# ZhendongWang6/Uformer

Hardware: AMD Instinct MI355X
Metric: restored images/sec (256x256, Uformer-B) (higher is better)
Workload: dtype bf16

## Files before the change

### include/uformer_hip.h

```cpp
#ifndef UFORMER_HIP_H
#define UFORMER_HIP_H

#include <stddef.h>
#include <stdint.h>

#ifdef __cplusplus
extern "C" {
#endif

#define UF_ABI_VERSION 1

typedef enum { UF_F32 = 0, UF_BF16 = 1, UF_F16 = 2 } uf_dtype;

#define UF_OK 0
#define UF_ERR_SHAPE (-1)
#define UF_ERR_UNSUPPORTED (-2)
#define UF_ERR_ALIGN (-3)
#define UF_ERR_LAUNCH (-4)
#define UF_ERR_WORKSPACE (-5)
#define UF_ERR_NULL (-6)

int uf_version(void);
int uf_last_error(char* buf, size_t n);

// ... 41 lines not shown
int uf_dwconv3x3_gelu_fwd(const void* x, const float* w9, const float* bias, void* out, int B,
                          int H, int W, int C, uf_dtype dtype, void* stream);
int uf_dwconv3x3_fwd(const void* x, const float* w9, const float* bias, void* out, int B, int H,
                     int W, int C, int gelu, uf_dtype dtype, void* stream);

int uf_dwconv3x3_pre_gelu_fwd(const void* x, const float* w9, const float* bias, void* pre_out, void* act_out, int B, int H,
                              int W, int C, uf_dtype dtype, void* stream);
int uf_dwconv3x3_gelu_in_pre_gelu_fwd(const void* pre_in, const float* w9, const float* bias, void* pre_out, void* act_out, int B, int H,
                                      int W, int C, uf_dtype dtype, void* stream);
int uf_dwconv3x3_mul_dgelu(const void* dy, const float* w9_flipped, const void* pre, void* out, int B, int H, int W, int C,
                           uf_dtype dtype, void* stream);

int uf_dwconv_linear2_fwd(const void* h1, const float* w9, const float* bdw, const void* W2_fm,
                          const float* b2, float* x, int ld, int B, int H, int W, int C,
                          uf_dtype dtype, void* stream);

typedef struct uf_block_params {
    const float* norm1_w;
    const float* norm1_b;
    const float* modulator;
    const float* rpb_dense;
    const float* rpb_fm;
    const float* rpb_tab;
    const void* wqkv_fm;
    const float* bqkv;
    const void* wproj;
    const void* wproj_fm;
    const float* bproj;
    const float* norm2_w;
    const float* norm2_b;
// ... 183 lines not shown
int uf_mixup(const float* x, float* out, const float* lam, const int* perm, int B, long long per_sample, void* stream);

typedef struct uf_model_desc {
    int32_t embed_dim, dd_in, in_chans;
    int32_t depths[9];
    const uf_block_params* blocks;
    const float* in_w27;
    const float* in_b;
    const float* out_w;
    const float* out_b;
    const void* down_w[4];
    const float* down_b[4];
    const void* up_w[4];
    const float* up_b[4];
    const void* down_w_fm[4];
} uf_model_desc;

size_t uf_uformer_workspace_bytes(const uf_model_desc* d, int B, int H, int W, uf_dtype dtype);
int uf_uformer_fwd(const uf_model_desc* d, const float* img, float* out, int B, int H, int W,
                   uf_dtype dtype, void* ws, size_t ws_bytes, void* stream);

typedef struct uf_block4_params {
    const float* norm1_w;  const float* norm1_b;  const float* norm2_w;  const float* norm2_b;
    const float* rpb4;
    const void* wqkv;
    const float* bqkv;
    const void* wproj;  const float* bproj;
    const void* w1;     const float* b1;
    const float* wdw9;  const float* bdw;
    const void* w2;     const float* b2;
// ... 46 lines not shown
```

### uformer_amd/_lib.py

```python
from __future__ import annotations

import ctypes as C
import os
import threading

_HERE = os.path.dirname(os.path.abspath(__file__))
LIB_PATH = os.path.join(_HERE, "lib", "libuformer_hip.so")
LIB_PATH = os.environ.get("UFORMER_HIP_LIB", LIB_PATH)

UF_F32, UF_BF16, UF_F16 = 0, 1, 2

c_int, c_void_p, c_size_t, c_float_p = C.c_int, C.c_void_p, C.c_size_t, C.c_void_p


class BlockParams(C.Structure):
    _fields_ = [(n, C.c_void_p) for n in (
        "norm1_w", "norm1_b", "modulator", "rpb_dense", "rpb_fm", "rpb_tab", "wqkv_fm", "bqkv", "wproj", "wproj_fm", "bproj",
        "norm2_w", "norm2_b", "w1_fm", "b1", "wdw9", "bdw", "w2_fm", "b2")] + [
        ("shift", C.c_int32), ("heads", C.c_int32), ("qkv_dw9", C.c_void_p), ("qkv_bdw", C.c_void_p)]


class BlockTrainParams(C.Structure):
    _fields_ = [(n, C.c_void_p) for n in (
        "norm1_w", "norm1_b", "norm2_w", "norm2_b", "modulator", "rpb_dense", "wqkv", "wqkv_t", "bqkv", "wproj", "wproj_t", "bproj",
# ... 14 lines not shown
class Block4Params(C.Structure):
    _fields_ = [(n, C.c_void_p) for n in (
        "norm1_w", "norm1_b", "norm2_w", "norm2_b", "rpb4", "wqkv", "bqkv", "wproj", "bproj", "w1", "b1", "wdw9", "bdw", "w2", "b2")] + [
        ("heads", C.c_int32)]


class ModelDesc(C.Structure):
    _fields_ = [
        ("embed_dim", C.c_int32), ("dd_in", C.c_int32), ("in_chans", C.c_int32),
        ("depths", C.c_int32 * 9),
        ("blocks", C.POINTER(BlockParams)),
        ("in_w27", C.c_void_p), ("in_b", C.c_void_p), ("out_w", C.c_void_p), ("out_b", C.c_void_p),
        ("down_w", C.c_void_p * 4), ("down_b", C.c_void_p * 4),
        ("up_w", C.c_void_p * 4), ("up_b", C.c_void_p * 4),
        ("down_w_fm", C.c_void_p * 4),
    ]


class UnetDesc(C.Structure):
    _fields_ = [
        ("dim", C.c_int32),
        ("in_w27", C.c_void_p), ("in_b", C.c_void_p), ("c11_w1", C.c_void_p), ("c11_b1", C.c_void_p),
        ("w0", C.c_void_p * 9), ("b0", C.c_void_p * 9), ("w2", C.c_void_p * 9), ("b2", C.c_void_p * 9),
        ("w11", C.c_void_p * 9), ("b11", C.c_void_p * 9),
        ("pool_w", C.c_void_p * 4), ("pool_b", C.c_void_p * 4), ("up_w", C.c_void_p * 4), ("up_b", C.c_void_p * 4),
        ("out_w", C.c_void_p), ("out_b", C.c_void_p),
    ]


P = c_void_p
# ... 28 lines not shown
    "uf_linear_residual_fwd": (I, [P, P, P, P, P, P, I, I, I, I, I, I, I, I, P]),
    "uf_layernorm_bwd_workspace_bytes": (c_size_t, [I, I]),
    "uf_layernorm_bwd": (I, [P, I, P, P, I, P, I, P, P, I, I, P, c_size_t, P]),
    "uf_layernorm_bwd_fused": (I, [P, I, P, P, I, I, P, P, I, P, P, I, I, I, I, I, I, I, P, c_size_t, P]),
    "uf_layernorm_bwd_cast": (I, [P, I, P, P, I, I, P, P, I, P, P, I, I, I, I, I, I, I, P, P, I, I, P, c_size_t, P]),
    "uf_linear_wgrad_workspace_bytes": (c_size_t, [I, I, I]),
    "uf_linear_wgrad": (I, [P, I, P, I, P, P, I, I, I, I, P, c_size_t, P]),
    "uf_window_attention_bwd_workspace_bytes": (c_size_t, [I, I]),
    "uf_window_attention_bwd": (I, [P, P, P, P, P, I, P, I, P, P, P, P, I, I, I, I, I, I, I, P, c_size_t, P]),
    "uf_window_attention_bwd_qkv": (I, [P, P, P, P, P, I, P, I, P, P, I, I, I, I, I, I, I, P, c_size_t, P]),
    "uf_dwconv3x3_wgrad_workspace_bytes": (c_size_t, [I, I]),
    "uf_dwconv3x3_wgrad": (I, [P, P, P, P, I, I, I, I, I, P, c_size_t, P]),
    "uf_dwconv3x3_bwd_workspace_bytes": (c_size_t, [I, I]),
    "uf_dwconv3x3_bwd": (I, [P, P, P, P, P, P, I, I, I, I, I, P, c_size_t, P]),
    "uf_dwconv_linear2_fwd": (I, [P, P, P, P, P, P, I, I, I, I, I, I, P]),
    "uf_block_workspace_bytes": (c_size_t, [I, I, I]),
    "uf_lewin_attn_fwd": (I, [C.POINTER(BlockParams), P, I, I, I, I, I, P, I, I, P, c_size_t, P]),
    "uf_leff_fwd": (I, [C.POINTER(BlockParams), P, I, I, I, I, I, I, P, c_size_t, P]),
    "uf_ffn_fwd": (I, [P, I, P, P, P, P, P, P, P, I, I, I, I, P]),
    "uf_mlp_fwd": (I, [C.POINTER(BlockParams), P, I, I, I, I, I, I, P, c_size_t, P]),
    "uf_lewin_attn_train_fwd": (I, [C.POINTER(BlockParams), P, I, P, I, I, I, I, I, P, I, P, P, P, P, P, P, P, P]),
    "uf_lewin_block_fwd": (I, [C.POINTER(BlockParams), P, I, I, I, I, I, P, I, I, P, c_size_t, P]),
    "uf_lewin_block_train_fwd": (I, [C.POINTER(BlockParams), P, I, I, I, I, I, P, P, I, P, c_size_t, P]),
    "uf_downsample_fwd": (I, [P, I, P, P, P, I, I, I, I, I, I, P]),
    "uf_downsample_fm_fwd": (I, [P, I, P, P, P, P, I, I, I, I, I, I, P]),
    "uf_upsample_fwd": (I, [P, I, P, P, P, I, I, I, I, I, I, I, P]),
    "uf_input_proj_fwd": (I, [P, P, P, P, I, I, I, I, I, I, P]),
    "uf_output_proj_fwd": (I, [P, I, P, P, P, P, I, I, I, I, I, P]),
    "uf_rows_sum_workspace_bytes": (c_size_t, [I, I]),
    "uf_rows_sum": (I, [P, I, P, I, I, I, P, c_size_t, P]),
# ... 95 lines not shown
```

### uformer_amd/csrc/uf_attnblk.hip

```cpp
#include <stdlib.h>

#include <atomic>
#include <type_traits>

#include "uf_internal.h"

namespace uf {
namespace {

struct AttnBlkParams {
    float* x; int ld;
    float* xo; int ldo;
    const float* gamma; const float* beta; const float* modulator;
    const void* Wqkv; const float* bqkv;
    const float* rpb_tab;
    const void* Wp; const float* bp;
    const float* gamma2; const float* beta2;
    const void* W1; const float* b1;
    void* h1;
    const float* drop;
    void* s_xn; void* s_q; void* s_k; void* s_vt; void* s_o; void* s_z;
    int n_windows, H, W, shift;
    float qscale;
    float qscale_plain;
// ... 2 lines not shown

constexpr float LOG2E = 1.4426950408889634f;

#ifndef UF_P1_OFFSET
#define UF_P1_OFFSET 0
#endif
#ifndef UF_FC1_OFFSET
#define UF_FC1_OFFSET 0
#endif
#ifndef UF_STAGGER
#define UF_STAGGER 0
#endif
#ifndef UF_SETPRIO
#define UF_SETPRIO 0
#endif
#define UF_PRIO_UP() do { if (UF_SETPRIO) __builtin_amdgcn_s_setprio(1); } while (0)
#define UF_PRIO_DN() do { if (UF_SETPRIO) __builtin_amdgcn_s_setprio(0); } while (0)
#ifndef UF_ABL
#define UF_ABL 0
#endif
#ifndef UF_NT
#define UF_NT 0
#endif
#ifndef UF_LN_ROTATE
#define UF_LN_ROTATE 0
#endif
#ifndef UF_LN_WIDE
#define UF_LN_WIDE 1
#endif
#ifndef UF_QKV_RING
// ... 796 lines not shown
    AttnBlkParams p{};
    p.drop = drop;
    p.x = x; p.ld = ld;
    p.xo = xo ? xo : x; p.ldo = xo ? ldo : ld; p.gamma = bp->norm1_w; p.beta = bp->norm1_b; p.modulator = bp->modulator;
    p.Wqkv = bp->wqkv_fm; p.bqkv = bp->bqkv; p.rpb_tab = bp->rpb_tab;
    p.Wp = bp->wproj_fm; p.bp = bp->bproj;
    p.gamma2 = bp->norm2_w; p.beta2 = bp->norm2_b; p.W1 = bp->w1_fm; p.b1 = bp->b1;
    p.h1 = dtype_half(dtype) ? h1_out : nullptr;
    p.n_windows = B * (H / 8) * (W / 8); p.H = H; p.W = W; p.shift = bp->shift;
    p.qscale = (float)(1.0 / sqrt(32.0)) * LOG2E;
    p.tbuf = debug_get_tbuf();

    const int forced = variant("attn", -1);
    const int lr = (forced >= 0 && forced <= 2) ? forced : (forced == 3 ? 0 : (C == 32 ? 2 : ((C == 128 && p.n_windows >= 4096) ? 1 : 0)));
    const bool st256 = forced == 3;
    const int nt_small = forced == 4 ? 64 : (forced == 5 ? 128 : ((forced < 0 && C == 32 && p.n_windows >= 8192) ? 64 : 0));
#define UF_AB(TT, CV, NTV) return launch_one<TT, CV, NTV>(p, st)
#define UF_AB_HALF(TT)                                                                                                              \
        switch (C) {                                                                                                                    \
            case 32:                                                                                                                    \
                if (nt_small == 64) return launch_one<TT, 32, 64, 0, 0, 4>(p, st);          \
                if (nt_small == 128) return launch_one<TT, 32, 128, 0, 0, 2>(p, st);                     \
                if (lr == 1) return launch_one<TT, 32, 256, 1>(p, st); if (lr == 2) return launch_one<TT, 32, 256, 2>(p, st); UF_AB(TT, 32, 256);      \
            case 64:                                                                                                                    \
                if (nt_small == 64) return launch_one<TT, 64, 64, 0, 0, 4>(p, st);             \
                if (nt_small == 128) return launch_one<TT, 64, 128, 0, 0, 4>(p, st);                            \
                if (lr == 1) return launch_one<TT, 64, 256, 1>(p, st); if (lr == 2) return launch_one<TT, 64, 256, 2>(p, st); UF_AB(TT, 64, 256);      \
            case 128: if (lr == 1) return launch_one<TT, 128, 256, 1>(p, st); if (lr == 2) return launch_one<TT, 128, 256, 2>(p, st); UF_AB(TT, 128, 256);                                                                                              \
            case 256:                                                                                                                   \
                if (p.n_windows <= 256) UF_AB(TT, 256, 512);    \
                if (st256) return launch_one<TT, 256, 256, 3>(p, st);          \
// ... 59 lines not shown
```

### uformer_amd/csrc/uf_internal.h

```cpp
#pragma once
#include "uf_common.h"

namespace uf {

enum ALoad { A_PLAIN = 0, A_FROM_R = 1, A_CONV_DOWN = 2 };
enum Epi {
    E_STORE_T = 0,
    E_STORE_T_GELU = 1,
    E_QKV = 2,
    E_RES_WINREV = 3,
    E_RES = 4,
    E_STORE_R = 5,
    E_UPSAMPLE = 6,
    E_STORE_T_PRE_GELU = 7,
    E_STORE_T_MUL_DGELU = 8
};

struct GemmParams {
    const void* A; int lda;
    const void* W;
    const void* W_fm = nullptr;
    const float* bias;
    int M, N, K;
    int H, W_, C;
// ... 10 lines not shown
int launch_down_dx(const void* dyT, int ld_dy, const void* w_pk_t, void* wc, float* dx, int ld_dx, int B, int H, int W, int Cin, int Cout, int accumulate, uf_dtype dtype,
                   hipStream_t st, bool* done);

constexpr int MAX_SIDE = 7, MAX_LANE_EVENTS = 8;
struct Lane { hipStream_t s[MAX_SIDE] = {}; hipEvent_t fork = nullptr, join[MAX_SIDE] = {}; int n = 0; hipEvent_t ev[MAX_LANE_EVENTS] = {}; int n_ev = 0; };
Lane* acquire_lane(int want, int* dev_out);
void release_lane(Lane* ln, int dev);
bool lane_events(Lane* ln, int want);

void debug_set_tbuf(void* p);
bool attn_block_supported(const uf_block_params* bp, const float* user_mask, uf_dtype dtype, int C, int heads);
int launch_attn_block(const uf_block_params* bp, float* x, int ld, int B, int H, int W, int C, uf_dtype dtype, void* h1_out, hipStream_t st,
                      const float* drop = nullptr, float* xo = nullptr, int ldo = 0);
int launch_leff2(const void* h1, const float* w9, const float* bdw, const void* W2, const float* b2, float* x, int ld, int B, int H, int W, int C,
                 uf_dtype dtype, const float* drop, hipStream_t st);

int launch_attn_block_train(const uf_block_params* bp, const float* x, int ld, float* x1, int ld1, int B, int H, int W, int C, uf_dtype dtype, const float* drop,
                            void* xn, void* q, void* k, void* vt, void* o, void* z, void* a1, hipStream_t st);

}
```

### uformer_amd/csrc/uf_leff2.hip

```cpp
#include <stdlib.h>

#include "uf_internal.h"
#include "uf_mconv.h"

namespace uf {
namespace {

struct Leff2Params {
    const void* h1;
    const float* w9; const float* bdw;
    const void* W2; const float* b2;
    float* x; int ld;
    const float* drop;
    int B, H, W;
    int n_tiles;
    unsigned long long* tbuf;
};

constexpr int KCW = 64;

#ifndef UF_MCONV
#define UF_MCONV 1
#endif
#ifndef UF_LEFF2_CP_DEFAULT
#define UF_LEFF2_CP_DEFAULT false
#endif
template <typename T> __device__ __forceinline__ void cvt8(const char* p, float* f);
template <> __device__ __forceinline__ void cvt8<bf16>(const char* p, float* f) { unpack8<bf16>(*reinterpret_cast<const u32x4*>(p), f); }
template <> __device__ __forceinline__ void cvt8<f16>(const char* p, float* f) { unpack8<f16>(*reinterpret_cast<const u32x4*>(p), f); }
template <> __device__ __forceinline__ void cvt8<float>(const char* p, float* f) {
    const f32x4 a = *reinterpret_cast<const f32x4*>(p), b = *reinterpret_cast<const f32x4*>(p + 16);
    f[0] = a[0]; f[1] = a[1]; f[2] = a[2]; f[3] = a[3]; f[4] = b[0]; f[5] = b[1]; f[6] = b[2]; f[7] = b[3];
}
__device__ __forceinline__ void put8(bf16* p, const float* f) { *reinterpret_cast<u32x4*>(p) = pack8<bf16>(f); }
__device__ __forceinline__ void put8(f16* p, const float* f) { *reinterpret_cast<u32x4*>(p) = pack8<f16>(f); }
__device__ __forceinline__ void put8(float* p, const float* f) {
    *reinterpret_cast<f32x4*>(p) = f32x4{f[0], f[1], f[2], f[3]};
    *reinterpret_cast<f32x4*>(p + 4) = f32x4{f[4], f[5], f[6], f[7]};
}

template <typename T, int C, int NPG, int NC, int NBUF, int WPS, int PW = 4, int CP = 0>
__global__ __launch_bounds__((PW * NPG + NC) * 64, WPS) void leff2_kernel(const Leff2Params p) {
    constexpr int NP = PW * NPG;
    constexpr int MC = sizeof(T) == 2 ? UF_MCONV : 0;
    static_assert(PW == 4 || (PW == 8 && MC != 0), "8 producer waves per group: MFMA stencil only (two pixel tiles per wave)");
    static_assert(CP == 0 || (MC != 0 && PW == 4 && NPG == 1 && NC == 4 * CP), "consumer stencil jobs: MFMA stencil, 4 producers, one job per consumer wave");
    constexpr int PTW = 16 / PW - CP;
    constexpr int SR = 2;
    constexpr int SZ = sizeof(T);
    constexpr int TH = 8, TW = 8, BM = 64;
    constexpr int HID = 4 * C;
    constexpr int KC = KCW * NPG;
    constexpr int NIT = HID / KC;
    static_assert(HID % KC == 0, "interval width");
    constexpr int HW_ = TW + 2, HT = (TH + 2) * HW_;
    constexpr int PS = KCW * SZ;
    constexpr int CPP = PS / 16;
    constexpr int HGB = (HT * PS + 1023) / 1024 * 1024;
    constexpr int NHG = HGB / 1024;
    constexpr int TRB = KC * 4;
    constexpr int TGB = (10 * TRB + 1023) / 1024 * 1024;
    constexpr int NTI = TGB / 1024;
    constexpr int NHI = NPG * NHG;
    constexpr int NI = NHI + NTI;
    constexpr int NS = (NI + NP - 1) / NP;
    constexpr int BUFB = NPG * HGB + TGB;
    constexpr int SAT = KC * SZ + 16;
    constexpr int AT_BYTES = BM * SAT;
    constexpr int WN = (C / 16) < NC ? (C / 16) : NC, WM = NC / WN;
    static_assert(WM <= 4, "consumer grid");
    constexpr int TMW = 4 / WM, TNW = (C / 16) / WN;
    extern __shared__ __attribute__((aligned(16))) char smem[];
    char* Ring = smem;
    char* At0 = smem + NBUF * BUFB;

    const int tid = threadIdx.x, lane = tid & 63;
    const int wave = __builtin_amdgcn_readfirstlane(tid >> 6);
    const bool producer = wave < NP;
    const int fr = lane & 15, fg = lane >> 4;
    const int tiles_x = p.W / TW, tiles_y = p.H / TH;
    const int G = (int)gridDim.x;
    const int nk = (p.n_tiles - (int)blockIdx.x + G - 1) / G;
    const int NTOT = nk * NIT;
    const int bt = xcd_tile(blockIdx.x, p.n_tiles);
    auto tile_coords = [&](int k, int& b, int& y0, int& x0) {
        const int t = xcd_tile((int)blockIdx.x + k * G, p.n_tiles);
// ... 134 lines not shown
    const int wlane = lane * 8 * SZ;
    auto w2_load = [&](int sub, int ks, int slot) {
#pragma unroll
        for (int i = 0; i < TNW; ++i) {
            const int soff = (((wn * TNW + i) * (HID / 32) + sub * 2 + ks) * 64) * 8 * SZ;
            if constexpr (SZ == 2) {
                wf[slot][i].v = __builtin_bit_cast(u32x4, __builtin_amdgcn_raw_buffer_load_b128(wrs, wlane, soff, 0));
            } else {
                wf[slot][i].lo = __builtin_bit_cast(f32x4, __builtin_amdgcn_raw_buffer_load_b128(wrs, wlane, soff, 0));
                wf[slot][i].hi = __builtin_bit_cast(f32x4, __builtin_amdgcn_raw_buffer_load_b128(wrs, wlane + 16, soff, 0));
            }
        }
    };
    auto w2_issue = [&](int sub) {
        if constexpr (WKS == 2) { w2_load(sub, 0, 0); w2_load(sub, 1, 1); }
    };

    f32x4 acc[TNW][TMW];
#pragma unroll
    for (int i = 0; i < TNW; ++i)
#pragma unroll
        for (int j = 0; j < TMW; ++j) acc[i][j] = f32x4{0.f, 0.f, 0.f, 0.f};

    constexpr bool XPRE = SZ == 2 && TNW * TMW <= 4 && CP == 0;
    f32x4 xres[XPRE ? TNW : 1][XPRE ? TMW : 1];
    auto x_ptr = [&](int b, int y0, int x0, int i, int j) -> float* {
        const int n = (wn * TNW + i) * 16 + fg * 4;
        const int pm = (wm * TMW + j) * 16 + fr;
        return p.x + ((size_t)(b * p.H + y0 + (pm >> 3)) * p.W + x0 + (pm & 7)) * p.ld + n;
    };
// ... 22 lines not shown
                for (int ks = 0; ks < 2; ++ks) {
                    if constexpr (WKS == 1) w2_load(sub, ks, 0);
                    Frag<T> af[TMW];
#pragma unroll
                    for (int jj = 0; jj < TMW; ++jj)
                        load_frag(af[jj], reinterpret_cast<const T*>(At + ((wm * TMW + jj) * 16 + fr) * SAT + (g * KCW + ks * 32 + fg * 8) * SZ));
                    __builtin_amdgcn_sched_barrier(0);
#pragma unroll
                    for (int ii = 0; ii < TNW; ++ii)
#pragma unroll
                        for (int jj = 0; jj < TMW; ++jj) mma16(acc[ii][jj], wf[WKS == 2 ? ks : 0][ii], af[jj]);
                    __builtin_amdgcn_sched_barrier(0);
                }
                if (sub + 1 < NIT * NPG) w2_issue(sub + 1);
                else if (j < NTOT) w2_issue(0);
                __builtin_amdgcn_sched_barrier(0);
            }
            if (it == NIT - 1) {
                const float dscale = p.drop ? p.drop[tb] : 1.0f;
#pragma unroll
                for (int i = 0; i < TNW; ++i) {
                    const f32x4 b2 = *reinterpret_cast<const f32x4*>(p.b2 + (wn * TNW + i) * 16 + fg * 4);
#pragma unroll
                    for (int jj = 0; jj < TMW; ++jj) {
                        float* xp = x_ptr(tb, ty0, tx0, i, jj);
                        f32x4 r;
                        if constexpr (XPRE) r = xres[i][jj]; else r = *reinterpret_cast<const f32x4*>(xp);
                        *reinterpret_cast<f32x4*>(xp) = r + (acc[i][jj] + b2) * dscale;
                        acc[i][jj] = f32x4{0.f, 0.f, 0.f, 0.f};
                    }
                }
            }
        }
        if constexpr (CP > 0) {
            if (j < NTOT) {
                const char* Hs = Ring + (j % NBUF) * BUFB;
                const float* Wl = reinterpret_cast<const float*>(Ring + (j % NBUF) * BUFB + NPG * HGB);
                mconv_job<T, MC, 1, KC, SAT, 2 * HW_ * PS>(Hs, Wl, At0 + (j & 1) * AT_BYTES, gq, 4 - CP + (cw >> 2), boff, msk, hshift, fr, fg);
            }
        }
        ct1 = __builtin_readcyclecounter(); ctw += ct1 - ct0; ct0 = ct1;
        lds_barrier();
        ct1 = __builtin_readcyclecounter(); ctbar += ct1 - ct0; ct0 = ct1;
    }
    if (p.tbuf && lane == 0 && (bt & 63) == 0) { p.tbuf[((bt >> 6) * 16 + wave) * 4] = ctw; p.tbuf[((bt >> 6) * 16 + wave) * 4 + 1] = ctbar; p.tbuf[((bt >> 6) * 16 + wave) * 4 + 2] = 0; }
    if (cw == 0 && lane == 0) {
        Census c2 = census;
        if (p.tbuf) { unsigned long long* o = p.tbuf + 65536 + (size_t)bt * 8; o[0] = c2.t0; o[1] = __builtin_readcyclecounter(); o[2] = c2.r0; o[3] = wall_clock64();
            o[4] = (unsigned long long)__builtin_amdgcn_s_getreg((31 << 11) | 4) | ((unsigned long long)__builtin_amdgcn_s_getreg((31 << 11) | 20) << 32); }
    }
}

template <typename T, int C, int NPG, int NC, int NBUF, int WPS, int PW = 4, int CP = 0>
int launch_v(const Leff2Params& p, hipStream_t st) {
    constexpr int SZ = sizeof(T), KC = KCW * NPG;
    constexpr int HGB = (100 * KCW * SZ + 1023) / 1024 * 1024, TGB = (10 * KC * 4 + 1023) / 1024 * 1024;
    constexpr int smem = NBUF * (NPG * HGB + TGB) + 2 * 64 * (KC * SZ + 16) + 1024;
    static_assert(smem <= 160 * 1024, "LDS budget");
    auto kern = leff2_kernel<T, C, NPG, NC, NBUF, WPS, PW, CP>;
    static bool lds_done[64] = {};
    if (int rc = ensure_dynamic_lds(reinterpret_cast<const void*>(kern), smem, lds_done, "leff2")) return rc;
    const long long M = (long long)p.B * p.H * p.W;
    char name[96] = "";
    if (timing_enabled()) snprintf(name, sizeof(name), "leff2_%s_c%d_np%d_nc%d %lldx%dx%d", TypeName<T>::s, C, PW * NPG, NC, M, C, 4 * C);
    {
        ScopedTimer tm(name, 2.0 * M * C * 4 * C + 18.0 * M * 4 * C, (double)M * 4 * C * SZ + (double)M * C * 8, st);
        const int pe = variant("persist", -1);
        const bool pays = C <= 32 || C >= 256 || (C == 128 && p.n_tiles <= 1024);
        const bool persist = pe >= 0 ? pe != 0 : pays;
        constexpr int waves = PW * NPG + NC;
        constexpr int by_lds = (160 * 1024) / smem, by_waves = 32 / waves, by_regs = (WPS * 4) / waves > 0 ? (WPS * 4) / waves : 1;
        constexpr int per_cu = by_lds < by_waves ? (by_lds < by_regs ? by_lds : by_regs) : (by_waves < by_regs ? by_waves : by_regs);
        const int resident = 256 * (per_cu < 1 ? 1 : per_cu);
        int grid = p.n_tiles;
        if (persist && p.n_tiles > resident) {
            const int rounds = (p.n_tiles + resident - 1) / resident;
            grid = ((p.n_tiles + rounds - 1) / rounds + 7) / 8 * 8;
        }
        hipLaunchKernelGGL(kern, dim3((unsigned)grid), dim3(waves * 64), smem, st, p);
    }
    return check_launch("leff2");
}

#ifndef UF_NB512
// ... 33 lines not shown
template <typename T>
int launch_t(const Leff2Params& p, int C, hipStream_t st) {
    switch (C) {
        case 16: return launch_c<T, 16>(p, st);
        case 32: return launch_c<T, 32>(p, st);
        case 64: return launch_c<T, 64>(p, st);
        case 128: return launch_c<T, 128>(p, st);
        case 256: return launch_c<T, 256>(p, st);
        case 512: return launch_c<T, 512>(p, st);
        default:
            set_error("leff2: C=%d unsupported (16,32,64,128,256,512)", C);
            return UF_ERR_UNSUPPORTED;
    }
}

}
unsigned long long* debug_get_tbuf();
}

using namespace uf;

namespace uf {
int launch_leff2(const void* h1, const float* w9, const float* bdw, const void* W2, const float* b2, float* x, int ld, int B, int H, int W, int C,
                 uf_dtype dtype, const float* drop, hipStream_t st) {
    UF_REQUIRE(h1 && w9 && bdw && W2 && b2 && x, UF_ERR_NULL, "uf_dwconv_linear2_fwd: null pointer");
    UF_REQUIRE(B > 0 && H >= 8 && W >= 8 && H % 8 == 0 && W % 8 == 0, UF_ERR_SHAPE, "uf_dwconv_linear2_fwd: B=%d H=%d W=%d (multiples of 8)", B, H, W);
    UF_REQUIRE(ld >= C && ld % 4 == 0, UF_ERR_ALIGN, "uf_dwconv_linear2_fwd: ld=%d", ld);
    UF_REQUIRE(((uintptr_t)h1 % 16) == 0 && ((uintptr_t)W2 % 16) == 0 && ((uintptr_t)x % 16) == 0 && ((uintptr_t)w9 % 16) == 0 &&
                   ((uintptr_t)bdw % 16) == 0 && ((uintptr_t)b2 % 16) == 0,
               UF_ERR_ALIGN, "uf_dwconv_linear2_fwd: operands must be 16-byte aligned");
    UF_REQUIRE((long long)H * W * 4LL * C * (long long)dtype_size(dtype) < 0xffffff00LL, UF_ERR_SHAPE,
               "uf_dwconv_linear2_fwd: one image of the hidden tensor must stay under 4 GiB (32-bit buffer offsets)");
    UF_REQUIRE((long long)B * H * W < 0x7fffffffLL / 4, UF_ERR_SHAPE, "uf_dwconv_linear2_fwd: too many tokens");
    Leff2Params p{};
    p.tbuf = debug_get_tbuf();
    p.h1 = h1; p.w9 = w9; p.bdw = bdw; p.W2 = W2; p.b2 = b2; p.x = x; p.ld = ld; p.B = B; p.H = H; p.W = W; p.drop = drop;
    p.n_tiles = B * (H / 8) * (W / 8);
    if (dtype == UF_BF16) return launch_t<bf16>(p, C, st);
    if (dtype == UF_F16) return launch_t<f16>(p, C, st);
    if (dtype == UF_F32) return launch_t<float>(p, C, st);
    set_error("uf_dwconv_linear2_fwd: dtype %d", (int)dtype);
    return UF_ERR_UNSUPPORTED;
}
}

extern "C" int uf_dwconv_linear2_fwd(const void* h1, const float* w9, const float* bdw, const void* W2, const float* b2,
                                     float* x, int ld, int B, int H, int W, int C, uf_dtype dtype, void* stream) {
    return uf::launch_leff2(h1, w9, bdw, W2, b2, x, ld, B, H, W, C, dtype, nullptr, (hipStream_t)stream);
}
```

### uformer_amd/csrc/uf_model.hip

```cpp
#include <stdlib.h>

#include <mutex>
#include <vector>

#include "uf_internal.h"

namespace uf {

int launch_layernorm(const float* x, int ld_x, const float* gamma, const float* beta, const float* modulator, void* out,
                     int rows, int H, int W, int C, int windowed, int shift, uf_dtype dtype, hipStream_t st);

int launch_unpack_weight_fm(const void* fm, void* w, int N, int K, uf_dtype dtype, hipStream_t st);

namespace {

struct BlockWs {
    char* a;
    char* h1;
    char* h2;
    char* wr;
};

bool wide_block(size_t C) { return C > 512; }

// ... 111 lines not shown
        rc = uf_dwconv3x3_gelu_fwd(w.h1, p->wdw9, p->bdw, w.h2, B, H, W, 4 * C, dtype, st);
        if (rc) return rc;
        rc = launch_unpack_weight_fm(p->w2_fm, w.wr, C, 4 * C, dtype, st);
        if (rc) return rc;
        GemmParams g{};
        g.A = w.h2; g.lda = 4 * C; g.W = w.wr; g.bias = p->b2; g.M = M; g.N = C; g.K = 4 * C;
        g.H = H; g.W_ = W; g.hw = H * W;
        g.out = x; g.ldo = ld; g.resid = x; g.ldr = ld;
        return launch_gemm(g, A_PLAIN, E_RES, dtype, st);
    }
    if (!fc1_done) {
        int rc = uf_ln_linear_gelu_fwd(x, ld, p->norm2_w, p->norm2_b, p->w1_fm, p->b1, w.h1, M, 4 * C, C, dtype, st);
        if (rc) return rc;
    }
    return launch_leff2(w.h1, p->wdw9, p->bdw, p->w2_fm, p->b2, x, ld, B, H, W, C, dtype, drop, st);
}

int block_fwd(const uf_block_params* p, float* x, int ld, int B, int H, int W, int C, const float* user_mask, int n_mask, uf_dtype dtype,
              const BlockWs& w, hipStream_t st, const float* drop_attn, const float* drop_leff) {
    bool fc1_done = false;
    int rc = attn_half(p, x, ld, B, H, W, C, user_mask, n_mask, dtype, w, st, &fc1_done, drop_attn);
    if (rc) return rc;
    return leff_half(p, x, ld, B, H, W, C, dtype, w, st, fc1_done, drop_leff);
}

}
}

using namespace uf;

// ... 172 lines not shown
    UF_REQUIRE(((uintptr_t)ws % 256) == 0, UF_ERR_ALIGN, "uf_uformer_fwd: workspace must be 256-byte aligned");
    UF_REQUIRE(ws_bytes >= pl.total, UF_ERR_WORKSPACE, "uf_uformer_fwd: workspace too small: %zu < %zu", ws_bytes, pl.total);
    UF_REQUIRE(d->in_chans == 3, UF_ERR_UNSUPPORTED, "uf_uformer_fwd: in_chans=%d (3 supported)", d->in_chans);
    hipStream_t st = (hipStream_t)stream;
    char* base = (char*)ws;
    float* D[4];
    for (int k = 0; k < 4; ++k) D[k] = (float*)(base + pl.off_D[k]);
    float* P = (float*)(base + pl.off_P);
    void* bws = base + pl.off_blk;

    auto enc_view = [&](int s, float*& ptr, int& ld) {
        ptr = D[3 - s] + pl.C[s];
        ld = 2 * pl.C[s];
    };
    const uf_block_params* blk = d->blocks;
    auto run_stage = [&](int s, float* x, int ld) -> int {
        for (int i = 0; i < d->depths[s]; ++i, ++blk) {
            int r = (s == 4 && bneck) ? uf_lewin_block4_fwd(bneck + i, x, ld, B, pl.res_h[s], pl.res_w[s], pl.C[s], nullptr, nullptr, dtype, bws, pl.blk_bytes, st)
                                      : uf_lewin_block_fwd(blk, x, ld, B, pl.res_h[s], pl.res_w[s], pl.C[s], nullptr, 0, dtype, bws, pl.blk_bytes, st);
            if (r) return r;
        }
        return UF_OK;
    };

    float* x; int ld;
    enc_view(0, x, ld);
    rc = uf_input_proj_fwd(img, d->in_w27, d->in_b, x, ld, B, d->dd_in, H, W, d->embed_dim, st);
    if (rc) return rc;
    for (int s = 0; s < 4; ++s) {
        rc = run_stage(s, x, ld);
        if (rc) return rc;
        float* nx; int nld;
        if (s < 3) enc_view(s + 1, nx, nld); else { nx = P; nld = pl.C[4]; }
        rc = uf_downsample_fm_fwd(x, ld, d->down_w[s], d->down_w_fm[s], d->down_b[s], nx, nld, B, pl.res_h[s], pl.res_w[s], pl.C[s], dtype, st);
        if (rc) return rc;
        x = nx; ld = nld;
    }
    rc = run_stage(4, x, ld);
    if (rc) return rc;
    for (int k = 0; k < 4; ++k) {
        const int s = 5 + k;
        const int cin = pl.C[s - 1], cout = pl.C[s] / 2;
        rc = uf_upsample_fwd(x, ld, d->up_w[k], d->up_b[k], D[k], pl.C[s], B, pl.res_h[s - 1], pl.res_w[s - 1], cin, cout, dtype, st);
        if (rc) return rc;
        x = D[k]; ld = pl.C[s];
        rc = run_stage(s, x, ld);
        if (rc) return rc;
    }
    return uf_output_proj_fwd(x, ld, d->out_w, d->out_b, img, out, B, H, W, pl.C[8], d->dd_in == 3 ? 1 : 0, st);
}

}

namespace {
int forward_split(const uf_model_desc* d, const uf_block4_params* bneck, const float* img, float* out, int B, int H, int W, uf_dtype dtype,
                  void* ws, size_t ws_bytes, void* stream) {
    static const int env_streams = getenv("UF_STREAMS") ? atoi(getenv("UF_STREAMS")) : 0;
    int n = env_streams > 0 ? (env_streams > MAX_SIDE + 1 ? MAX_SIDE + 1 : env_streams) : (B >= 8 ? 2 : 1);
    if (n > B) n = B;
    if (n < 2 || timing_enabled()) return forward_one_stream(d, bneck, img, out, B, H, W, dtype, ws, ws_bytes, stream);
    UF_REQUIRE(d && img && out && ws, UF_ERR_NULL, "uf_uformer_fwd: null pointer");
// ... 47 lines not shown
```

### uformer_amd/packing.py

```python
from __future__ import annotations

import ctypes as C
from typing import Dict, List

import torch

from . import _lib

Tensor = torch.Tensor


def rpb_dense(table: Tensor, index: Tensor) -> Tensor:
    n = index.shape[0]
    return table.detach()[index.reshape(-1)].reshape(n, n, -1).permute(2, 0, 1).contiguous().float()


def pack_frag(w: Tensor, dtype: torch.dtype) -> Tensor:
    N, K = w.shape
    KP = (K + 31) // 32 * 32
    w = w.detach().to(dtype)
    if KP != K:
        w = torch.nn.functional.pad(w, (0, KP - K))
    return w.reshape(N // 16, 16, KP // 32, 4, 8).permute(0, 2, 3, 1, 4).contiguous()

# ... 167 lines not shown
        }
        for name, tns in g.items():
            setattr(d, name, tns.data_ptr())
        self.keep.append(g)
        for k in range(4):
            dw = pack_downsample(sd[f"dowsample_{k}.conv.0.weight"], dtype)
            db = sd[f"dowsample_{k}.conv.0.bias"].detach().float().clone().contiguous()
            uw = pack_upsample(sd[f"upsample_{k}.deconv.0.weight"], dtype)
            ub = sd[f"upsample_{k}.deconv.0.bias"].detach().float().clone().contiguous()
            d.down_w[k], d.down_b[k], d.up_w[k], d.up_b[k] = dw.data_ptr(), db.data_ptr(), uw.data_ptr(), ub.data_ptr()
            dwf = None
            if dtype in (torch.bfloat16, torch.float16) and dw.is_cuda and dw.shape[0] % 16 == 0 and dw.shape[1] % 32 == 0:
                from . import ops
                dwf = ops.pack_weight_fm(dw)
            d.down_w_fm[k] = dwf.data_ptr() if dwf is not None else None
            self.keep.append((dw, db, uw, ub, dwf))
        self.desc = d


def pack_conv(w: Tensor, dtype: torch.dtype) -> Tensor:
    cout, cin, k, _ = w.shape
    cp, np_ = (cin + 31) // 32 * 32, (cout + 63) // 64 * 64
    t = torch.zeros(np_, k, k, cp, dtype=dtype, device=w.device)
    t[:cout, :, :, :cin] = w.detach().permute(0, 2, 3, 1).to(dtype)
    return t.reshape(np_, -1).contiguous()


def pack_conv_dgrad(w: Tensor, dtype: torch.dtype) -> Tensor:
    return pack_conv(w.detach().transpose(0, 1).flip(2, 3), dtype)


# ... 31 lines not shown
```

Before: 2539.

## Fuse decoder upsample into last block's dwconv+linear2 kernel

Adds a leff2 kernel variant that computes the block's output residual into LDS and then runs the 2x2 transposed-conv upsample GEMM in the same kernel, writing the upsampled tensor directly. This removes the round trip of the stage output through global memory and a separate upsample launch. By default it is enabled only for the C=512, Cout=128 case. It also adds an optional wave-64 attention tile choice for C=64, which is off by default. The fused path skips the write of the block output to x and disables persistent scheduling for this kernel.

```diff
diff --git a/include/uformer_hip.h b/include/uformer_hip.h
--- a/include/uformer_hip.h
+++ b/include/uformer_hip.h
@@ -79,6 +79,9 @@
 int uf_dwconv_linear2_fwd(const void* h1, const float* w9, const float* bdw, const void* W2_fm,
                           const float* b2, float* x, int ld, int B, int H, int W, int C,
                           uf_dtype dtype, void* stream);
+int uf_dwconv_linear2_upsample_fwd(const void* h1, const float* w9, const float* bdw, const void* W2_fm, const float* b2, const float* x, int ld,
+                                   const void* up_w_fm, const float* up_b, float* out, int ld_o, int B, int H, int W, int C, int Cout,
+                                   uf_dtype dtype, void* stream);
 
 typedef struct uf_block_params {
     const float* norm1_w;
@@ -292,6 +295,7 @@
     const void* up_w[4];
     const float* up_b[4];
     const void* down_w_fm[4];
+    const void* up_w_fm[4];
 } uf_model_desc;
 
 size_t uf_uformer_workspace_bytes(const uf_model_desc* d, int B, int H, int W, uf_dtype dtype);
diff --git a/uformer_amd/_lib.py b/uformer_amd/_lib.py
--- a/uformer_amd/_lib.py
+++ b/uformer_amd/_lib.py
@@ -52,6 +52,7 @@
         ("down_w", C.c_void_p * 4), ("down_b", C.c_void_p * 4),
         ("up_w", C.c_void_p * 4), ("up_b", C.c_void_p * 4),
         ("down_w_fm", C.c_void_p * 4),
+        ("up_w_fm", C.c_void_p * 4),
     ]
 
 
@@ -110,6 +111,7 @@
     "uf_dwconv3x3_bwd_workspace_bytes": (c_size_t, [I, I]),
     "uf_dwconv3x3_bwd": (I, [P, P, P, P, P, P, I, I, I, I, I, P, c_size_t, P]),
     "uf_dwconv_linear2_fwd": (I, [P, P, P, P, P, P, I, I, I, I, I, I, P]),
+    "uf_dwconv_linear2_upsample_fwd": (I, [P, P, P, P, P, P, I, P, P, P, I, I, I, I, I, I, I, P]),
     "uf_block_workspace_bytes": (c_size_t, [I, I, I]),
     "uf_lewin_attn_fwd": (I, [C.POINTER(BlockParams), P, I, I, I, I, I, P, I, I, P, c_size_t, P]),
     "uf_leff_fwd": (I, [C.POINTER(BlockParams), P, I, I, I, I, I, I, P, c_size_t, P]),
diff --git a/uformer_amd/csrc/uf_attnblk.hip b/uformer_amd/csrc/uf_attnblk.hip
--- a/uformer_amd/csrc/uf_attnblk.hip
+++ b/uformer_amd/csrc/uf_attnblk.hip
@@ -40,6 +40,9 @@
 #ifndef UF_SETPRIO
 #define UF_SETPRIO 0
 #endif
+#ifndef UF_ATTN_WAVE64
+#define UF_ATTN_WAVE64 0
+#endif
 #define UF_PRIO_UP() do { if (UF_SETPRIO) __builtin_amdgcn_s_setprio(1); } while (0)
 #define UF_PRIO_DN() do { if (UF_SETPRIO) __builtin_amdgcn_s_setprio(0); } while (0)
 #ifndef UF_ABL
@@ -866,7 +869,8 @@
     const int forced = variant("attn", -1);
     const int lr = (forced >= 0 && forced <= 2) ? forced : (forced == 3 ? 0 : (C == 32 ? 2 : ((C == 128 && p.n_windows >= 4096) ? 1 : 0)));
     const bool st256 = forced == 3;
-    const int nt_small = forced == 4 ? 64 : (forced == 5 ? 128 : ((forced < 0 && C == 32 && p.n_windows >= 8192) ? 64 : 0));
+    const bool wave_shape = (C == 32 || (UF_ATTN_WAVE64 && C == 64)) && p.n_windows >= 8192;
+    const int nt_small = forced == 4 ? 64 : (forced == 5 ? 128 : ((forced < 0 && wave_shape) ? 64 : 0));
 #define UF_AB(TT, CV, NTV) return launch_one<TT, CV, NTV>(p, st)
 #define UF_AB_HALF(TT)                                                                                                              \
         switch (C) {                                                                                                                    \
diff --git a/uformer_amd/csrc/uf_internal.h b/uformer_amd/csrc/uf_internal.h
--- a/uformer_amd/csrc/uf_internal.h
+++ b/uformer_amd/csrc/uf_internal.h
@@ -48,6 +48,7 @@
                       const float* drop = nullptr, float* xo = nullptr, int ldo = 0);
 int launch_leff2(const void* h1, const float* w9, const float* bdw, const void* W2, const float* b2, float* x, int ld, int B, int H, int W, int C,
                  uf_dtype dtype, const float* drop, hipStream_t st);
+bool leff2_upsample_supported(int C, int Cout, uf_dtype dtype);
 
 int launch_attn_block_train(const uf_block_params* bp, const float* x, int ld, float* x1, int ld1, int B, int H, int W, int C, uf_dtype dtype, const float* drop,
                             void* xn, void* q, void* k, void* vt, void* o, void* z, void* a1, hipStream_t st);
diff --git a/uformer_amd/csrc/uf_leff2.hip b/uformer_amd/csrc/uf_leff2.hip
--- a/uformer_amd/csrc/uf_leff2.hip
+++ b/uformer_amd/csrc/uf_leff2.hip
@@ -16,6 +16,12 @@
     int n_tiles;
     unsigned long long* tbuf;
 };
+struct Leff2UpParams : Leff2Params {
+    const void* up_w; const float* up_b;
+    float* out; int ld_o;
+};
+template <int UP> struct ParamsOf { typedef Leff2UpParams type; };
+template <> struct ParamsOf<0> { typedef Leff2Params type; };
 
 constexpr int KCW = 64;
 
@@ -39,8 +45,8 @@
     *reinterpret_cast<f32x4*>(p + 4) = f32x4{f[4], f[5], f[6], f[7]};
 }
 
-template <typename T, int C, int NPG, int NC, int NBUF, int WPS, int PW = 4, int CP = 0>
-__global__ __launch_bounds__((PW * NPG + NC) * 64, WPS) void leff2_kernel(const Leff2Params p) {
+template <typename T, int C, int NPG, int NC, int NBUF, int WPS, int PW = 4, int CP = 0, int UP = 0>
+__global__ __launch_bounds__((PW * NPG + NC) * 64, WPS) void leff2_kernel(const typename ParamsOf<UP>::type p) {
     constexpr int NP = PW * NPG;
     constexpr int MC = sizeof(T) == 2 ? UF_MCONV : 0;
     static_assert(PW == 4 || (PW == 8 && MC != 0), "8 producer waves per group: MFMA stencil only (two pixel tiles per wave)");
@@ -70,6 +76,12 @@
     constexpr int WN = (C / 16) < NC ? (C / 16) : NC, WM = NC / WN;
     static_assert(WM <= 4, "consumer grid");
     constexpr int TMW = 4 / WM, TNW = (C / 16) / WN;
+    constexpr int SXT = C * SZ + 16, XT_BYTES = BM * SXT;
+    constexpr int BASE_BYTES = NBUF * BUFB + 2 * AT_BYTES + 1024;
+    constexpr int XT_OFF = XT_BYTES <= NBUF * BUFB ? 0 : BASE_BYTES;
+    constexpr int SRB = TNW * 64 + 16, STG_W = 16 * SRB, STG_OFF = XT_OFF == 0 ? XT_BYTES : 0;
+    static_assert(UP == 0 || (SZ == 2 && WM == 1 && CP == 0 && NPG == 1 && (UP * C) % 4 == 0), "fused Upsample: 2-byte operands, every consumer wave owns all 64 pixels");
+    static_assert(UP == 0 || STG_OFF + NC * STG_W <= BASE_BYTES, "fused Upsample: staging tiles");
     extern __shared__ __attribute__((aligned(16))) char smem[];
     char* Ring = smem;
     char* At0 = smem + NBUF * BUFB;
@@ -234,6 +246,19 @@
     };
     auto w2_issue = [&](int sub) {
         if constexpr (WKS == 2) { w2_load(sub, 0, 0); w2_load(sub, 1, 1); }
+    };
+    constexpr int UQ = C / 64, UTOT = UP * UQ;
+    __amdgpu_buffer_rsrc_t urs;
+    if constexpr (UP > 0) urs = __builtin_amdgcn_make_buffer_rsrc(const_cast<void*>(p.up_w), 0, UP * C * C * SZ, 0x00020000);
+    auto up_load = [&](int g, int ks, int slot) {
+        if constexpr (UP > 0 && SZ == 2) {
+            const int ps = g / UQ, q = g - ps * UQ;
+#pragma unroll
+            for (int i = 0; i < TNW; ++i) {
+                const int soff = (((ps * (C / 16) + wn * TNW + i) * (C / 32) + q * 2 + ks) * 64) * 8 * SZ;
+                wf[slot][i].v = __builtin_bit_cast(u32x4, __builtin_amdgcn_raw_buffer_load_b128(urs, wlane, soff, 0));
+            }
+        }
     };
 
     f32x4 acc[TNW][TMW];
@@ -286,6 +311,7 @@
                 }
                 if (sub + 1 < NIT * NPG) w2_issue(sub + 1);
                 else if (j < NTOT) w2_issue(0);
+                else if constexpr (UP > 0) { up_load(0, 0, 0); up_load(0, 1, 1); }
                 __builtin_amdgcn_sched_barrier(0);
             }
             if (it == NIT - 1) {
@@ -298,6 +324,10 @@
                         float* xp = x_ptr(tb, ty0, tx0, i, jj);
                         f32x4 r;
                         if constexpr (XPRE) r = xres[i][jj]; else r = *reinterpret_cast<const f32x4*>(xp);
+                        if constexpr (UP > 0) {
+                            const f32x4 v = r + (acc[i][jj] + b2) * dscale;
+                            store4(reinterpret_cast<T*>(smem + XT_OFF + ((wm * TMW + jj) * 16 + fr) * SXT) + (wn * TNW + i) * 16 + fg * 4, v);
+                        } else
                         *reinterpret_cast<f32x4*>(xp) = r + (acc[i][jj] + b2) * dscale;
                         acc[i][jj] = f32x4{0.f, 0.f, 0.f, 0.f};
                     }
@@ -315,6 +345,57 @@
         lds_barrier();
         ct1 = __builtin_readcyclecounter(); ctbar += ct1 - ct0; ct0 = ct1;
     }
+    if constexpr (UP > 0 && SZ == 2) {
+        constexpr int CO = UP * C / 4;
+        constexpr int CPR = TNW * 4, RPI = 64 / CPR;
+        int tb, ty0, tx0;
+        tile_coords(0, tb, ty0, tx0);
+        const char* Xt = smem + XT_OFF;
+        char* stg = smem + STG_OFF + cw * STG_W;
+#pragma unroll 1
+        for (int g = 0; g < UTOT; ++g) {
+#pragma unroll
+            for (int ks = 0; ks < 2; ++ks) {
+                Frag<T> af[TMW];
+#pragma unroll
+                for (int jj = 0; jj < TMW; ++jj)
+                    load_frag(af[jj], reinterpret_cast<const T*>(Xt + (jj * 16 + fr) * SXT + ((g % UQ) * 64 + ks * 32 + fg * 8) * SZ));
+                __builtin_amdgcn_sched_barrier(0);
+#pragma unroll
+                for (int ii = 0; ii < TNW; ++ii)
+#pragma unroll
+                    for (int jj = 0; jj < TMW; ++jj) mma16(acc[ii][jj], wf[ks][ii], af[jj]);
+                __builtin_amdgcn_sched_barrier(0);
+                if (g + 1 < UTOT) up_load(g + 1, ks, ks);
+                __builtin_amdgcn_sched_barrier(0);
+            }
+            if (g % UQ == UQ - 1) {
+                const int nb = (g / UQ) * C + wn * TNW * 16;
+                f32x4 bv[TNW];
+#pragma unroll
+                for (int i = 0; i < TNW; ++i) bv[i] = *reinterpret_cast<const f32x4*>(p.up_b + (nb + i * 16 + fg * 4) % CO);
+#pragma unroll
+                for (int jj = 0; jj < TMW; ++jj) {
+#pragma unroll
+                    for (int i = 0; i < TNW; ++i) {
+                        *reinterpret_cast<f32x4*>(stg + fr * SRB + (i * 16 + fg * 4) * 4) = acc[i][jj] + bv[i];
+                        acc[i][jj] = f32x4{0.f, 0.f, 0.f, 0.f};
+                    }
+                    asm volatile("s_waitcnt lgkmcnt(0)" ::: "memory");
+#pragma unroll
+                    for (int it = 0; it < 16 / RPI; ++it) {
+                        const int r = it * RPI + lane / CPR, cb = lane % CPR;
+                        const f32x4 val = *reinterpret_cast<const f32x4*>(stg + r * SRB + cb * 16);
+                        const int pm = jj * 16 + r, n2 = nb + cb * 4;
+                        const int qd = n2 / CO, co = n2 - qd * CO;
+                        const size_t row = (size_t)(tb * 2 * p.H + 2 * (ty0 + (pm >> 3)) + (qd >> 1)) * (size_t)(2 * p.W) + 2 * (tx0 + (pm & 7)) + (qd & 1);
+                        *reinterpret_cast<f32x4*>(p.out + row * p.ld_o + co) = val;
+                    }
+                    asm volatile("s_waitcnt lgkmcnt(0)" ::: "memory");
+                }
+            }
+        }
+    }
     if (p.tbuf && lane == 0 && (bt & 63) == 0) { p.tbuf[((bt >> 6) * 16 + wave) * 4] = ctw; p.tbuf[((bt >> 6) * 16 + wave) * 4 + 1] = ctbar; p.tbuf[((bt >> 6) * 16 + wave) * 4 + 2] = 0; }
     if (cw == 0 && lane == 0) {
         Census c2 = census;
@@ -323,23 +404,25 @@
     }
 }
 
-template <typename T, int C, int NPG, int NC, int NBUF, int WPS, int PW = 4, int CP = 0>
-int launch_v(const Leff2Params& p, hipStream_t st) {
+template <typename T, int C, int NPG, int NC, int NBUF, int WPS, int PW = 4, int CP = 0, int UP = 0>
+int launch_v(const typename ParamsOf<UP>::type& p, hipStream_t st) {
     constexpr int SZ = sizeof(T), KC = KCW * NPG;
     constexpr int HGB = (100 * KCW * SZ + 1023) / 1024 * 1024, TGB = (10 * KC * 4 + 1023) / 1024 * 1024;
-    constexpr int smem = NBUF * (NPG * HGB + TGB) + 2 * 64 * (KC * SZ + 16) + 1024;
+    constexpr int ring = NBUF * (NPG * HGB + TGB), xt = 64 * (C * SZ + 16);
+    constexpr int smem = ring + 2 * 64 * (KC * SZ + 16) + 1024 + ((UP > 0 && xt > ring) ? xt : 0);
     static_assert(smem <= 160 * 1024, "LDS budget");
-    auto kern = leff2_kernel<T, C, NPG, NC, NBUF, WPS, PW, CP>;
+    auto kern = leff2_kernel<T, C, NPG, NC, NBUF, WPS, PW, CP, UP>;
     static bool lds_done[64] = {};
     if (int rc = ensure_dynamic_lds(reinterpret_cast<const void*>(kern), smem, lds_done, "leff2")) return rc;
     const long long M = (long long)p.B * p.H * p.W;
     char name[96] = "";
-    if (timing_enabled()) snprintf(name, sizeof(name), "leff2_%s_c%d_np%d_nc%d %lldx%dx%d", TypeName<T>::s, C, PW * NPG, NC, M, C, 4 * C);
+    if (timing_enabled()) snprintf(name, sizeof(name), "leff2%s_%s_c%d_np%d_nc%d %lldx%dx%d", UP > 0 ? (UP == 2 ? "_up2" : "_up1") : "", TypeName<T>::s, C, PW * NPG, NC, M, C, 4 * C);
     {
-        ScopedTimer tm(name, 2.0 * M * C * 4 * C + 18.0 * M * 4 * C, (double)M * 4 * C * SZ + (double)M * C * 8, st);
+        ScopedTimer tm(name, 2.0 * M * C * 4 * C + 18.0 * M * 4 * C + (UP > 0 ? 2.0 * M * UP * C * C : 0.0),
+                       (double)M * 4 * C * SZ + (UP > 0 ? (double)M * C * 4 + (double)M * UP * C * 4 + (double)UP * C * C * SZ : (double)M * C * 8), st);
         const int pe = variant("persist", -1);
         const bool pays = C <= 32 || C >= 256 || (C == 128 && p.n_tiles <= 1024);
-        const bool persist = pe >= 0 ? pe != 0 : pays;
+        const bool persist = UP > 0 ? false : (pe >= 0 ? pe != 0 : pays);
         constexpr int waves = PW * NPG + NC;
         constexpr int by_lds = (160 * 1024) / smem, by_waves = 32 / waves, by_regs = (WPS * 4) / waves > 0 ? (WPS * 4) / waves : 1;
         constexpr int per_cu = by_lds < by_waves ? (by_lds < by_regs ? by_lds : by_regs) : (by_waves < by_regs ? by_waves : by_regs);
@@ -403,6 +486,29 @@
     }
 }
 
+template <typename T, int C, int UP>
+int launch_cu(const Leff2UpParams& p, hipStream_t st) {
+    if constexpr (C == 128) {
+        if (p.n_tiles <= 1024) return launch_v<T, C, 1, 4, 2, 6, 8, 0, UP>(p, st);
+        return launch_v<T, C, 1, 4, 2, 6, 4, 0, UP>(p, st);
+    } else if constexpr (C == 256) {
+        if (p.n_tiles <= 256) return launch_v<T, C, 1, 8, UF_NB256E, 4, 8, 0, UP>(p, st);
+        return launch_v<T, C, 1, 4, UF_NB256, 4, 4, 0, UP>(p, st);
+    } else {
+        return launch_v<T, C, 1, 8, UF_NB512, 3, 4, 0, UP>(p, st);
+    }
+}
+
+template <typename T>
+int launch_tu(const Leff2UpParams& p, int C, int N, hipStream_t st) {
+    if (C == 128 && N == 128) return launch_cu<T, 128, 1>(p, st);
+    if (C == 256 && N == 256) return launch_cu<T, 256, 1>(p, st);
+    if (C == 512 && N == 512) return launch_cu<T, 512, 1>(p, st);
+    if (C == 512 && N == 1024) return launch_cu<T, 512, 2>(p, st);
+    set_error("uf_dwconv_linear2_upsample_fwd: (C, 4 Cout) = (%d, %d) is not built: (128, 128), (256, 256), (512, 512), (512, 1024)", C, N);
+    return UF_ERR_UNSUPPORTED;
+}
+
 }
 unsigned long long* debug_get_tbuf();
 }
@@ -410,6 +516,10 @@
 using namespace uf;
 
 namespace uf {
+bool leff2_upsample_supported(int C, int Cout, uf_dtype dtype) {
+    return dtype_half(dtype) && ((C == 128 && Cout == 32) || (C == 256 && Cout == 64) || (C == 512 && (Cout == 128 || Cout == 256)));
+}
+
 int launch_leff2(const void* h1, const float* w9, const float* bdw, const void* W2, const float* b2, float* x, int ld, int B, int H, int W, int C,
                  uf_dtype dtype, const float* drop, hipStream_t st) {
     UF_REQUIRE(h1 && w9 && bdw && W2 && b2 && x, UF_ERR_NULL, "uf_dwconv_linear2_fwd: null pointer");
@@ -433,6 +543,31 @@
 }
 }
 
+extern "C" int uf_dwconv_linear2_upsample_fwd(const void* h1, const float* w9, const float* bdw, const void* W2, const float* b2, const float* x, int ld,
+                                              const void* up_w_fm, const float* up_b, float* out, int ld_o, int B, int H, int W, int C, int Cout,
+                                              uf_dtype dtype, void* stream) {
+    UF_REQUIRE(h1 && w9 && bdw && W2 && b2 && x && up_w_fm && up_b && out, UF_ERR_NULL, "uf_dwconv_linear2_upsample_fwd: null pointer");
+    UF_REQUIRE(B > 0 && H >= 8 && W >= 8 && H % 8 == 0 && W % 8 == 0, UF_ERR_SHAPE, "uf_dwconv_linear2_upsample_fwd: B=%d H=%d W=%d (multiples of 8)", B, H, W);
+    UF_REQUIRE(dtype_half(dtype), UF_ERR_UNSUPPORTED, "uf_dwconv_linear2_upsample_fwd: dtype %d (bf16 / f16 operands)", (int)dtype);
+    UF_REQUIRE(C > 0 && Cout > 0 && leff2_upsample_supported(C, Cout, dtype), UF_ERR_UNSUPPORTED,
+               "uf_dwconv_linear2_upsample_fwd: (C, 4 Cout) = (%d, %d) is not built: (128, 128), (256, 256), (512, 512), (512, 1024)", C, 4 * Cout);
+    UF_REQUIRE(ld >= C && ld % 4 == 0 && ld_o >= Cout && ld_o % 4 == 0, UF_ERR_ALIGN, "uf_dwconv_linear2_upsample_fwd: ld=%d ld_o=%d", ld, ld_o);
+    UF_REQUIRE(((uintptr_t)h1 % 16) == 0 && ((uintptr_t)W2 % 16) == 0 && ((uintptr_t)x % 16) == 0 && ((uintptr_t)w9 % 16) == 0 &&
+                   ((uintptr_t)bdw % 16) == 0 && ((uintptr_t)b2 % 16) == 0 && ((uintptr_t)up_w_fm % 16) == 0 && ((uintptr_t)up_b % 16) == 0 &&
+                   ((uintptr_t)out % 16) == 0,
+               UF_ERR_ALIGN, "uf_dwconv_linear2_upsample_fwd: operands must be 16-byte aligned");
+    UF_REQUIRE((long long)H * W * 4LL * C * (long long)dtype_size(dtype) < 0xffffff00LL, UF_ERR_SHAPE,
+               "uf_dwconv_linear2_upsample_fwd: one image of the hidden tensor must stay under 4 GiB (32-bit buffer offsets)");
+    UF_REQUIRE((long long)B * H * W < 0x7fffffffLL / 16, UF_ERR_SHAPE, "uf_dwconv_linear2_upsample_fwd: too many tokens");
+    Leff2UpParams p{};
+    p.tbuf = debug_get_tbuf();
+    p.h1 = h1; p.w9 = w9; p.bdw = bdw; p.W2 = W2; p.b2 = b2; p.x = const_cast<float*>(x); p.ld = ld; p.B = B; p.H = H; p.W = W; p.drop = nullptr;
+    p.n_tiles = B * (H / 8) * (W / 8);
+    p.up_w = up_w_fm; p.up_b = up_b; p.out = out; p.ld_o = ld_o;
+    if (dtype == UF_BF16) return launch_tu<bf16>(p, C, 4 * Cout, (hipStream_t)stream);
+    return launch_tu<f16>(p, C, 4 * Cout, (hipStream_t)stream);
+}
+
 extern "C" int uf_dwconv_linear2_fwd(const void* h1, const float* w9, const float* bdw, const void* W2, const float* b2,
                                      float* x, int ld, int B, int H, int W, int C, uf_dtype dtype, void* stream) {
     return uf::launch_leff2(h1, w9, bdw, W2, b2, x, ld, B, H, W, C, dtype, nullptr, (hipStream_t)stream);
diff --git a/uformer_amd/csrc/uf_model.hip b/uformer_amd/csrc/uf_model.hip
--- a/uformer_amd/csrc/uf_model.hip
+++ b/uformer_amd/csrc/uf_model.hip
@@ -149,6 +149,24 @@
         if (rc) return rc;
     }
     return launch_leff2(w.h1, p->wdw9, p->bdw, p->w2_fm, p->b2, x, ld, B, H, W, C, dtype, drop, st);
+}
+
+bool block_takes_upsample(const uf_block_params* p, int C, int Cout, uf_dtype dtype) {
+    return !mlp_block(p) && !conv_block(p) && !wide_block((size_t)C) && leff2_upsample_supported(C, Cout, dtype);
+}
+
+bool upsample_fusion_pays(int C, int Cout) { return C == 512 && Cout == 128; }
+
+int block_upsample_fwd(const uf_block_params* p, float* x, int ld, int B, int H, int W, int C, uf_dtype dtype, const BlockWs& w, hipStream_t st,
+                       const void* up_w_fm, const float* up_b, float* out, int ld_o, int Cout) {
+    bool fc1_done = false;
+    int rc = attn_half(p, x, ld, B, H, W, C, nullptr, 0, dtype, w, st, &fc1_done, nullptr);
+    if (rc) return rc;
+    if (!fc1_done) {
+        rc = uf_ln_linear_gelu_fwd(x, ld, p->norm2_w, p->norm2_b, p->w1_fm, p->b1, w.h1, B * H * W, 4 * C, C, dtype, st);
+        if (rc) return rc;
+    }
+    return uf_dwconv_linear2_upsample_fwd(w.h1, p->wdw9, p->bdw, p->w2_fm, p->b2, x, ld, up_w_fm, up_b, out, ld_o, B, H, W, C, Cout, dtype, st);
 }
 
 int block_fwd(const uf_block_params* p, float* x, int ld, int B, int H, int W, int C, const float* user_mask, int n_mask, uf_dtype dtype,
@@ -351,8 +369,22 @@
         ld = 2 * pl.C[s];
     };
     const uf_block_params* blk = d->blocks;
-    auto run_stage = [&](int s, float* x, int ld) -> int {
+    const int upfuse = variant("upfuse", 1);
+    auto run_stage = [&](int s, float* x, int ld, int up = -1, bool* fused = nullptr) -> int {
         for (int i = 0; i < d->depths[s]; ++i, ++blk) {
+            if (up >= 0 && i == d->depths[s] - 1 && !(s == 4 && bneck) && d->up_w_fm[up] && upfuse != 0 &&
+                (upfuse == 2 || upsample_fusion_pays(pl.C[s], pl.C[s + 1] / 2)) && block_takes_upsample(blk, pl.C[s], pl.C[s + 1] / 2, dtype)) {
+                int r = check_block_args(blk, x, ld, B, pl.res_h[s], pl.res_w[s], pl.C[s], dtype);
+                if (r) return r;
+                BlockWs w;
+                r = carve(w, bws, pl.blk_bytes, pl.M[s], pl.C[s], dtype);
+                if (r) return r;
+                r = block_upsample_fwd(blk, x, ld, B, pl.res_h[s], pl.res_w[s], pl.C[s], dtype, w, st, d->up_w_fm[up], d->up_b[up], D[up], pl.C[s + 1],
+                                       pl.C[s + 1] / 2);
+                if (r) return r;
+                *fused = true;
+                continue;
+            }
             int r = (s == 4 && bneck) ? uf_lewin_block4_fwd(bneck + i, x, ld, B, pl.res_h[s], pl.res_w[s], pl.C[s], nullptr, nullptr, dtype, bws, pl.blk_bytes, st)
                                       : uf_lewin_block_fwd(blk, x, ld, B, pl.res_h[s], pl.res_w[s], pl.C[s], nullptr, 0, dtype, bws, pl.blk_bytes, st);
             if (r) return r;
@@ -373,15 +405,19 @@
         if (rc) return rc;
         x = nx; ld = nld;
     }
-    rc = run_stage(4, x, ld);
+    bool up_done = false;
+    rc = run_stage(4, x, ld, 0, &up_done);
     if (rc) return rc;
     for (int k = 0; k < 4; ++k) {
         const int s = 5 + k;
         const int cin = pl.C[s - 1], cout = pl.C[s] / 2;
-        rc = uf_upsample_fwd(x, ld, d->up_w[k], d->up_b[k], D[k], pl.C[s], B, pl.res_h[s - 1], pl.res_w[s - 1], cin, cout, dtype, st);
-        if (rc) return rc;
+        if (!up_done) {
+            rc = uf_upsample_fwd(x, ld, d->up_w[k], d->up_b[k], D[k], pl.C[s], B, pl.res_h[s - 1], pl.res_w[s - 1], cin, cout, dtype, st);
+            if (rc) return rc;
+        }
         x = D[k]; ld = pl.C[s];
-        rc = run_stage(s, x, ld);
+        up_done = false;
+        rc = k < 3 ? run_stage(s, x, ld, k + 1, &up_done) : run_stage(s, x, ld);
         if (rc) return rc;
     }
     return uf_output_proj_fwd(x, ld, d->out_w, d->out_b, img, out, B, H, W, pl.C[8], d->dd_in == 3 ? 1 : 0, st);
diff --git a/uformer_amd/packing.py b/uformer_amd/packing.py
--- a/uformer_amd/packing.py
+++ b/uformer_amd/packing.py
@@ -205,7 +205,12 @@
                 from . import ops
                 dwf = ops.pack_weight_fm(dw)
             d.down_w_fm[k] = dwf.data_ptr() if dwf is not None else None
-            self.keep.append((dw, db, uw, ub, dwf))
+            uwf = None
+            if dtype in (torch.bfloat16, torch.float16) and uw.is_cuda and uw.shape[0] % 16 == 0 and uw.shape[1] % 32 == 0:
+                from . import ops
+                uwf = ops.pack_weight_fm(uw)
+            d.up_w_fm[k] = uwf.data_ptr() if uwf is not None else None
+            self.keep.append((dw, db, uw, ub, dwf, uwf))
         self.desc = d
 
 
```

Result: no change. 2561, median of 6 (+0.8%).
